# 9to1url/PairPhone

Hardware: AMD Instinct MI355X
Metric: MELPe-1200 channel-seconds encoded/sec (node) (higher is better)
Workload: dtype int16/int32 saturating fixed point; 1 GPU; config 4: 262144 channels per GPU, melpe_a per superframe (NPP x3 + MELPe-1200 analysis + 81-bit packing); channels_per_gpu=262144, channels_total=262144, parallelism=channel shards, 1 GPU(s), no collective

## Files before the change

### pairphone_amd/csrc/k_npp.hip

```cpp
#ifndef MELPE_NPP_WG_WAVES
#define MELPE_NPP_WG_WAVES 1
#endif
#ifndef MELPE_NPP_MATH_LDS
#define MELPE_NPP_MATH_LDS 1
#endif
#if MELPE_NPP_MATH_LDS
#define MELPE_MATH_LDS
#endif
#include "kern.h"
#include "npp_wave.h"
#include "dsp_eval.h"

MELPE_TU(npp)

#define NPP_WG (WAVE * MELPE_NPP_WG_WAVES)
#if MELPE_NPP_MATH_LDS
static_assert((160 * 1024 / (MELPE_NPP_WG_WAVES * sizeof(mlp::wv::NppWave) + MTAB_WORDS * sizeof(int16_t))) *
			      MELPE_NPP_WG_WAVES >= 16,
	      "16 NPP waves per CU (the register budget's four per SIMD)");
#define NPP_LDS_DYN (MTAB_WORDS * sizeof(int16_t))
#define NPP_TABLES_IN()                                                        \
	do {                                                                   \
		for (int i_ = threadIdx.x; i_ < MTAB_WORDS; i_ += blockDim.x) \
			s_mtab[i_] = g_tab[mtab_src(i_)];                     \
		__syncthreads();                                               \
	} while (0)
#else
#define NPP_LDS_DYN 0
#define NPP_TABLES_IN() (void) 0
#endif

#ifndef NPP_WAVES_PER_EU
#define NPP_WAVES_PER_EU 4
#endif
#define NPP_WPE __attribute__((amdgpu_waves_per_eu(NPP_WAVES_PER_EU)))

using namespace mlp::wv;

__global__ __launch_bounds__(NPP_WG) NPP_WPE void k_npp(EncState *enc, int16_t *sp, int frames, int stride,
					      const uint8_t *active, int n, int rate1200)
{
	__shared__ NppWave Ws[MELPE_NPP_WG_WAVES];
	NPP_TABLES_IN();
	const int w = __builtin_amdgcn_readfirstlane(threadIdx.x / WAVE), lane = threadIdx.x % WAVE;
	const int c = blockIdx.x * MELPE_NPP_WG_WAVES + w;
	if (c >= n || (active && !active[c]))
		return;
	NppWave &W = Ws[w];
	WvConst kc;
	wv_const_init(&kc, lane);
	wv_state_in(&W, &enc[c].npp, lane);
	int16_t *x = sp + (size_t) c * stride;
	for (int f = 0; f < frames; f++)
		wv_npp_frame(&W, &enc[c].npp, x + f * NPP_HOP, stride - f * NPP_HOP, rate1200 != 0, &kc, lane);
	wv_state_out(&enc[c].npp, &W, lane);
}

__global__ __launch_bounds__(NPP_WG) NPP_WPE void k_enc_npp(EncState *enc, int16_t *sp, const uint8_t *active,
						  int n)
{
	__shared__ NppWave Ws[MELPE_NPP_WG_WAVES];
	NPP_TABLES_IN();
	const int w = __builtin_amdgcn_readfirstlane(threadIdx.x / WAVE), lane = threadIdx.x % WAVE;
	const int c = blockIdx.x * MELPE_NPP_WG_WAVES + w;
	if (c >= n || (active && !active[c]))
		return;
	NppWave &W = Ws[w];
	WvConst kc;
	wv_const_init(&kc, lane);
	wv_state_in(&W, &enc[c].npp, lane);
	int16_t *x = sp + (size_t) c * BLOCK;
	for (int f = 0; f < NF; f++)
		wv_npp_frame(&W, &enc[c].npp, x + f * FRAME, BLOCK - f * FRAME, true, &kc, lane);
	wv_state_out(&enc[c].npp, &W, lane);
}

static unsigned npp_grid(int n)
{
	return (unsigned) ((n + MELPE_NPP_WG_WAVES - 1) / MELPE_NPP_WG_WAVES);
}

extern "C" int kl_npp(EncState *enc, int16_t *sp, int frames, int stride, const uint8_t *active,
		      int n, int rate1200, hipStream_t s)
{
	k_npp<<<npp_grid(n), NPP_WG, NPP_LDS_DYN, s>>>(enc, sp, frames, stride, active, n, rate1200);
	return (int) hipGetLastError();
}

static int launch_enc_npp(int waves, EncState *enc, int16_t *sp, const uint8_t *active, int n, hipStream_t s)
{
	k_enc_npp<<<npp_grid(waves), NPP_WG, NPP_LDS_DYN, s>>>(enc, sp, active, n);
	return (int) hipGetLastError();
}

extern "C" int kl_enc_npp(EncState *enc, int16_t *sp, const uint8_t *active, int n, hipStream_t s)
{
	return launch_enc_npp(n, enc, sp, active, n, s);
}

extern "C" size_t kl_npp_private(void)
{
	const size_t x = private_bytes((const void *) k_enc_npp), y = private_bytes((const void *) k_npp);
	return x > y ? x : y;
}

extern "C" int kl_npp_warm(int n, hipStream_t s)
{
	return launch_enc_npp(n, nullptr, nullptr, nullptr, 0, s);
}

__global__ __launch_bounds__(NPP_WG) void k_dsp_scalar_lds(int mode, const int32_t *args, int32_t *out, long n)
{
	NPP_TABLES_IN();
	long i = blockIdx.x * (long) blockDim.x + threadIdx.x;
	if (i >= n)
		return;
	const int32_t *a = args + 4 * i;
	out[i] = de_scalar(mode, a[0], a[1], a[2], a[3]);
}

__global__ __launch_bounds__(NPP_WG) void k_dsp_wave_fft(int mode, const int16_t *in, const int32_t *args,
							  int32_t *out, int n)
{
	__shared__ int16_t d[MELPE_NPP_WG_WAVES][DE_WV_IN];
	NPP_TABLES_IN();
	const int w = __builtin_amdgcn_readfirstlane(threadIdx.x / WAVE), lane = threadIdx.x % WAVE;
	const int c = blockIdx.x * MELPE_NPP_WG_WAVES + w;
	if (c >= n)
		return;
	WvConst kc;
	wv_const_init(&kc, lane);
	LANE_LOOP(k, DE_WV_IN)
		d[w][k] = in[(size_t) c * DE_WV_IN + k];
	wsync();
	const Word16 g = mode == 1 ? wv_fft_npp(d[w], (Word16) args[4 * (size_t) c], &kc, lane)
				   : wv_cfft256(d[w], &kc, lane);
	int32_t *o = out + (size_t) c * DE_WV_OUT;
	if (lane < DE_RET)
		o[lane] = lane == 0 ? g : 0;
	LANE_LOOP(k, DE_WV_IN)
		o[DE_RET + k] = d[w][k];
}

extern "C" int kl_dsp_scalar_lds(int mode, const int32_t *args, int32_t *out, long n, hipStream_t s)
{
	k_dsp_scalar_lds<<<(unsigned) ((n + NPP_WG - 1) / NPP_WG), NPP_WG, NPP_LDS_DYN, s>>>(mode, args, out, n);
	return (int) hipGetLastError();
}

extern "C" int kl_dsp_wave_fft(int mode, const int16_t *in, const int32_t *args, int32_t *out, int n,
			       hipStream_t s)
{
	k_dsp_wave_fft<<<npp_grid(n), NPP_WG, NPP_LDS_DYN, s>>>(mode, in, args, out, n);
	return (int) hipGetLastError();
}
```

### pairphone_amd/csrc/npp.h

```cpp
#ifndef MELPE_NPP_H
#define MELPE_NPP_H

#include <stddef.h>

#include "dsp.h"

namespace mlp {

#define NPP_WIN 256
#define NPP_HOP 180
#define NPP_OVL 76
#define NPP_NB 129
#define NPP_NMINWIN 8
#define NPP_LMINWIN 9
#define GM_MIN 3932
#define ENH_QK_MAX 32735
#define ENH_QK_MIN 33
#define NOISE_BIAS 23170

struct NppState {
	int16_t started;
	int16_t qk_started;
	int16_t pf_started;
	int16_t enh_i;
// ... 460 lines not shown
	}
	s1 = sub(norm_l(L), 1);
	Word16 t1 = extract_h(L_shl(L, s1));
	Word16 t = sub(sub(s4, s1), ns2_shift);
	w->var_rel[i] = divide_s(t1, ns2);
	if (cmp_shift(w->var_rel[i], t, 16384, 0) > 0)
		w->var_rel[i] = 16384;
	else
		w->var_rel[i] = shl(w->var_rel[i], t);
	if (w->var_rel[i] < 0)
		w->var_rel[i] = 0;
}

template <class SC>
MD Word16 npp_bias_scalars(NppState *s, const SC *w, Word32 vsum, Word16 *f1, Word16 *f2)
{
	vsum = L_shl(vsum, 1);
	vsum = L_sub(vsum, L_deposit_l(w->var_rel[0]));
	vsum = L_sub(vsum, L_deposit_l(w->var_rel[NPP_NB - 1]));
	s->var_rel_av = extract_l(L_shr(vsum, 8));
	if (s->var_rel_av < 0)
		s->var_rel_av = 0;
	Word16 vsq = mult(12288, sqrt_Q15(s->var_rel_av));
	vsq = add(8192, vsq);
	*f1 = extract_h(L_shl(L_mult(vsq, 16521), 1));
	*f2 = extract_h(L_shl(L_mult(vsq, 18643), 1));
	return vsq;
}

template <class SC>
MD void npp_bias2_bin(const NppState *s, const SC *w, int16_t &bsp, int16_t &bsh,
		      int16_t &bsub, int16_t &bsubsh, Word16 vsq, Word16 f1, Word16 f2, int i)
{
	Word32 L3 = L_mult(vsq, s->smoothedspect[i]);
	Word16 vr = w->var_rel[i];
	Word32 L4 = L_mult(vr, s->smoothedspect[i]);
	Word16 t = add(19543, shr(vr, 1));
	t = add(11656, shr(mult(vr, t), 1));
	Word32 L = L_mpy_ls(L_mpy_ls(L4, f1), t);
	L = L_add(L_shr(L3, 6), L_shr(L, 1));
	if (L < 1)
		L = 1;
	Word16 s1 = norm_l(L);
	bsp = extract_h(L_shl(L, s1));
	bsh = add(s->sm_shift[i], sub(8, s1));
	t = add(13968, shr(vr, 2));
	t = add(11909, shr(mult(vr, t), 1));
	L = L_mpy_ls(L_mpy_ls(L4, f2), t);
	L = L_add(L_shr(L3, 4), L_shr(L, 1));
	if (L < 1)
		L = 1;
	s1 = norm_l(L);
	bsub = extract_h(L_shl(L, s1));
	bsubsh = add(s->sm_shift[i], sub(6, s1));
}

MN void npp_bias_compensation(NppState *s, NppScratch *w, int16_t *bsp, int16_t *bsh,
			      int16_t *bsub, int16_t *bsubsh)
{
	Word32 vsum = 0;
	for (int i = 0; i < NPP_NB; i++) {
		npp_bias1_bin(s, w, i, w->alpha_var[i], w->noisespect2[i], w->noise2_shift[i]);
		vsum = L_add(vsum, L_deposit_l(w->var_rel[i]));
	}
	Word16 f1, f2;
	Word16 vsq = npp_bias_scalars(s, w, vsum, &f1, &f2);
	for (int i = 0; i < NPP_NB; i++)
		npp_bias2_bin(s, w, bsp[i], bsh[i], bsub[i], bsubsh[i], vsq, f1, f2, i);
}

MD Word16 npp_noise_slope(const NppState *s)
{
	if (s->var_rel_av > 5898)
		return 2703;
	if (s->var_rel_av < 983 || s->enh_i < 50)
		return 18022;
	if (s->var_rel_av < 1638)
		return 9011;
	if (s->var_rel_av < 1966)
		return 4506;
	return 2703;
}

MD void npp_min_search_bin(NppState *s, NppState *m, int16_t bsp, int16_t bsh, int16_t bsub,
			   int16_t bsubsh, Word16 slope, int i)
{
	if (s->minspec_counter == 0) {
		if (cmp_shift(bsp, bsh, s->act_min[i], s->act_min_shift[i]) < 0) {
			s->act_min[i] = bsp;
			s->act_min_shift[i] = bsh;
			m->act_min_sub[i] = bsub;
			m->act_min_sub_shift[i] = bsubsh;
			m->localflag[i] = 0;
		}
		m->circb[s->circb_index][i] = s->act_min[i];
		m->circb_shift[s->circb_index][i] = s->act_min_shift[i];
		Word16 t1 = m->circb[0][i], t2 = m->circb_shift[0][i];
		for (int k = 1; k < NPP_NMINWIN; k++)
			if (cmp_shift(m->circb[k][i], m->circb_shift[k][i], t1, t2) < 0) {
				t1 = m->circb[k][i];
				t2 = m->circb_shift[k][i];
			}
		m->circb_min[i] = t1;
		m->circb_min_shift[i] = t2;
		Word16 t = mult(slope, m->circb_min[i]);
		Word16 ts = add(m->circb_min_shift[i], 4);
		if (m->localflag[i] &&
		    cmp_shift(m->act_min_sub[i], m->act_min_sub_shift[i],
			      m->circb_min[i], m->circb_min_shift[i]) > 0 &&
		    cmp_shift(m->act_min_sub[i], m->act_min_sub_shift[i], t, ts) < 0) {
			m->circb_min[i] = m->act_min_sub[i];
			m->circb_min_shift[i] = m->act_min_sub_shift[i];
			for (int k = 0; k < NPP_NMINWIN; k++) {
				m->circb[k][i] = m->circb_min[i];
				m->circb_shift[k][i] = m->circb_min_shift[i];
			}
		}
		m->localflag[i] = 0;
	} else if (s->minspec_counter == 1) {
		s->act_min[i] = bsp;
		s->act_min_shift[i] = bsh;
		m->act_min_sub[i] = bsub;
		m->act_min_sub_shift[i] = bsubsh;
	} else {
		if (cmp_shift(bsp, bsh, s->act_min[i], s->act_min_shift[i]) < 0) {
			s->act_min[i] = bsp;
			s->act_min_shift[i] = bsh;
			m->act_min_sub[i] = bsub;
			m->act_min_sub_shift[i] = bsubsh;
			m->localflag[i] = 1;
		}
		if (cmp_shift(m->act_min_sub[i], m->act_min_sub_shift[i],
			      m->circb_min[i], m->circb_min_shift[i]) < 0) {
			m->circb_min[i] = m->act_min_sub[i];
			m->circb_min_shift[i] = m->act_min_sub_shift[i];
		}
		s->noisespect[i] = m->circb_min[i];
		s->noise_shift[i] = m->circb_min_shift[i];
		Word32 L = L_mult(NOISE_BIAS, s->noisespect[i]);
		if (L < 0x40000000L) {
			L = L_shl(L, 1);
			s->lambdaD_shift[i] = s->noise_shift[i];
		} else {
			s->lambdaD_shift[i] = add(s->noise_shift[i], 1);
		}
		s->lambdaD[i] = extract_h(L);
	}
}

MD void npp_min_search_post(NppState *s)
{
	if (s->minspec_counter == 0) {
		s->circb_index = add(s->circb_index, 1);
		if (s->circb_index == NPP_NMINWIN)
			s->circb_index = 0;
	}
	s->minspec_counter = add(s->minspec_counter, 1);
	if (s->minspec_counter == NPP_LMINWIN)
		s->minspec_counter = 0;
}

MN void npp_min_search(NppState *s, const int16_t *bsp, const int16_t *bsh,
		       const int16_t *bsub, const int16_t *bsubsh)
{
	Word16 slope = npp_noise_slope(s);
	for (int i = 0; i < NPP_NB; i++)
		npp_min_search_bin(s, s, bsp[i], bsh[i], bsub[i], bsubsh[i], slope, i);
	npp_min_search_post(s);
}

MN void npp_minstat_init(NppState *s)
{
	v_copy(s->smoothedspect, s->lambdaD, NPP_NB);
	v_scale(s->smoothedspect, NOISE_BIAS, NPP_NB);
	for (int k = 0; k < NPP_NMINWIN; k++) {
		v_copy(s->circb[k], s->smoothedspect, NPP_NB);
		v_copy(s->circb_shift[k], s->lambdaD_shift, NPP_NB);
	}
	v_copy(s->sm_shift, s->lambdaD_shift, NPP_NB);
	v_copy(s->act_min, s->smoothedspect, NPP_NB);
	v_copy(s->act_min_shift, s->lambdaD_shift, NPP_NB);
	v_copy(s->act_min_sub, s->smoothedspect, NPP_NB);
	v_copy(s->act_min_sub_shift, s->lambdaD_shift, NPP_NB);
	v_copy(s->noisespect, s->smoothedspect, NPP_NB);
	v_copy(s->noise_shift, s->lambdaD_shift, NPP_NB);
	for (int i = 0; i < NPP_NB; i++) {
		s->var_sp_av[i] = mult(s->smoothedspect[i], 20066);
		s->av_shift[i] = add(s->lambdaD_shift[i], 1);
		Word32 L = L_mult(s->smoothedspect[i], s->smoothedspect[i]);
		Word16 sh = norm_l(L);
		s->var_sp_2[i] = extract_h(L_shl(L, sh));
		s->av2_shift[i] = sub(shl(s->lambdaD_shift[i], 1), sub(sh, 1));
	}
	s->alphacorr = 29491;
}

MN void npp_enh_init(NppState *s, NppScratch *w, int16_t *noise)
{
	int16_t *yb = w->ybuf;
	int32_t ty[NPP_WIN + 2];
	window(noise, TB(sqrt_tukey_256_180), noise, NPP_WIN);
	Word16 mx = 1;
	for (int i = 0; i < NPP_WIN; i++) {
		Word16 t = abs_s(noise[i]);
		if (t > mx)
			mx = t;
	}
	Word16 sh = norm_s(mx);
	Word16 ash = sub(15, sh);
	v_zero(yb, 2 * NPP_WIN + 2);
	for (int i = 0; i < NPP_WIN; i++)
		yb[2 * i] = shl(noise[i], sh);
	Word16 g = fft_npp(yb, 1);
	ty[0] = L_shr(L_mult(yb[0], yb[0]), 1);
	ty[1] = 0;
	ty[NPP_WIN] = L_shr(L_mult(yb[NPP_WIN], yb[NPP_WIN]), 1);
	ty[NPP_WIN + 1] = 0;
	for (int i = 2; i < NPP_WIN - 1; i += 2) {
		ty[i + 1] = 0;
		ty[i] = L_shr(L_add(L_mult(yb[i], yb[i]), L_mult(yb[i + 1], yb[i + 1])), 1);
	}
	Word32 L = ty[0];
	for (int i = 1; i < NPP_WIN + 1; i++)
		if (L < ty[i])
			L = ty[i];
	sh = norm_l(L);
	for (int i = 0; i < NPP_WIN + 1; i++)
		yb[i] = extract_h(L_shl(ty[i], sh));
	sh = sub(shl(add(ash, g), 1), add(sh, 7));
	for (int i = 0; i < NPP_WIN / 2 - 1; i++) {
// ... 352 lines not shown
```

### pairphone_amd/csrc/npp_wave.h

```cpp
#ifndef MELPE_NPP_WAVE_H
#define MELPE_NPP_WAVE_H

#include "npp.h"

namespace mlp {
namespace wv {

#define WV 64
#define LANE_LOOP(i, n) for (int i = lane; i < (n); i += WV)
#define BIN_LOOP(t, i) \
	_Pragma("unroll") for (int t = 0, i = lane; t < 3; t++, i += WV) if (i < NPP_NB)

#define BIN_PASSES(t, i, ...) \
	_Pragma("unroll") for (int t = 0, i = lane; t < 3; t++, i += WV) if (i < NPP_NB) { \
		__VA_ARGS__ \
	}
__device__ __forceinline__ void wsync()
{
#if defined(MELPE_NPP_WG_WAVES) && MELPE_NPP_WG_WAVES > 1
	__builtin_amdgcn_fence(__ATOMIC_RELEASE, "wavefront");
	__builtin_amdgcn_wave_barrier();
	__builtin_amdgcn_fence(__ATOMIC_ACQUIRE, "wavefront");
#else
	__syncthreads();
// ... 171 lines not shown
		o[6] = sub(v[2], v[7]);
		o[3] = sub(v[3], v[6]);
		o[7] = add(v[3], v[6]);
		m = 0;
		for (int k = 0; k < 8; k++) {
			d0[i + k] = o[k];
			m = max(m, (int) abs_s(o[k]));
		}
	}
	int16_t *d = d0 - 1;
	int st = 0;
#pragma unroll
	for (int mmax = 8; mmax < 512; mmax *= 2, st++) {
		Word16 mx = (Word16) wmax(m);
		sc = 0;
		if (mx > 16383) {
			g += 2;
			sc = 2;
		} else if (mx > 8191) {
			g += 1;
			sc = 1;
		}
		wsync();
		int istep = 2 * mmax;
		int half = mmax / 2;
		m = 0;
		for (int t = 0; t < 2; t++) {
			int b = lane + WV * t;
			int k = b % half, blk = b / half;
			int i = 1 + 2 * k + blk * istep;
			int jj = i + mmax;
			Word16 wr = (Word16) (kc->tw[st][t] & 0xffff);
			Word16 wi = (Word16) (kc->tw[st][t] >> 16);
			Word16 pr = shr(d[i], sc), qr = shr(d[jj], sc);
			Word16 pi = shr(d[i + 1], sc), qi = shr(d[jj + 1], sc);
			Word32 tr = L_add(L_mult(wr, qr), L_mult(wi, qi));
			tr = L_add(tr, L_shl(0x80, 8));
			tr = L_shl(L_shr(tr, 16), 16);
			Word32 ti = L_sub(L_mult(wi, qr), L_mult(wr, qi));
			ti = L_add(ti, L_shl(0x80, 8));
			ti = L_shl(L_shr(ti, 16), 16);
			Word16 o0 = extract_h(L_add(L_deposit_h(pr), tr));
			Word16 o1 = extract_h(L_sub(L_deposit_h(pr), tr));
			Word16 o2 = extract_h(L_sub(L_deposit_h(pi), ti));
			Word16 o3 = extract_h(L_add(L_deposit_h(pi), ti));
			d[i] = o0;
			d[jj] = o1;
			d[i + 1] = o2;
			d[jj + 1] = o3;
			m = max(m, max(max((int) abs_s(o0), (int) abs_s(o1)),
				       max((int) abs_s(o2), (int) abs_s(o3))));
		}
	}
	wsync();
	return g;
}

MD Word16 wv_fft_npp(int16_t *d, Word16 dir, const WvConst *kc, int lane)
{
	Word16 g = wv_cfft256(d, kc, lane);
	if (dir < 0) {
		for (int n = 1 + lane; n < 128; n += WV) {
			int16_t t = d[2 * n];
			d[2 * n] = d[2 * (256 - n)];
			d[2 * (256 - n)] = t;
			t = d[2 * n + 1];
			d[2 * n + 1] = d[2 * (256 - n) + 1];
			d[2 * (256 - n) + 1] = t;
		}
		wsync();
	}
	return g;
}

MD void wv_mirror(int16_t *yb, int lane)
{
	LANE_LOOP(i, NPP_WIN / 2 - 1) {
		yb[NPP_WIN + 2 * i + 2] = yb[NPP_WIN - 2 * i - 2];
		yb[NPP_WIN + 2 * i + 3] = negate(yb[NPP_WIN - 2 * i - 1]);
	}
	wsync();
}

MD void wv_minstat_init(NppState *s, NppState *m, int lane)
{
	LANE_LOOP(i, NPP_NB) {
		Word16 sp = mult(s->lambdaD[i], NOISE_BIAS);
		Word16 ls = s->lambdaD_shift[i];
		s->smoothedspect[i] = sp;
		for (int k = 0; k < NPP_NMINWIN; k++) {
			m->circb[k][i] = sp;
			m->circb_shift[k][i] = ls;
		}
		s->sm_shift[i] = ls;
		s->act_min[i] = sp;
		s->act_min_shift[i] = ls;
		m->act_min_sub[i] = sp;
		m->act_min_sub_shift[i] = ls;
		s->noisespect[i] = sp;
		s->noise_shift[i] = ls;
		s->var_sp_av[i] = mult(sp, 20066);
		s->av_shift[i] = add(ls, 1);
		Word32 L = L_mult(sp, sp);
		Word16 sh = norm_l(L);
		s->var_sp_2[i] = extract_h(L_shl(L, sh));
		s->av2_shift[i] = sub(shl(ls, 1), sub(sh, 1));
	}
	s->alphacorr = 29491;
}

MD void wv_enh_init(NppWave *W, int16_t *noise, const WvConst *kc, int lane, NppState *m)
{
	NppState *s = wv_S(W);
	int16_t *yb = W->w.ybuf;
	u32_alias *ty = W->ty_init;
	int mx = 0;
#pragma unroll
	LANE_LOOP(i, NPP_WIN) {
		noise[i] = mult(kc->win[i >> 6], noise[i]);
		mx = max(mx, (int) abs_s(noise[i]));
	}
	mx = max(1, wmax(mx));
	Word16 sh = norm_s((Word16) mx);
	Word16 ash = sub(15, sh);
	LANE_LOOP(i, NPP_WIN + 1) {
		yb[2 * i] = (i < NPP_WIN) ? shl(noise[i], sh) : (int16_t) 0;
		yb[2 * i + 1] = 0;
	}
	wsync();
	Word16 g = wv_fft_npp(yb, 1, kc, lane);
	int Lm = INT32_MIN;
	LANE_LOOP(p, NPP_NB) {
		int i = 2 * p;
		Word32 v;
		if (p == 0 || p == NPP_NB - 1)
			v = L_shr(L_mult(yb[i], yb[i]), 1);
		else
			v = L_shr(L_add(L_mult(yb[i], yb[i]), L_mult(yb[i + 1], yb[i + 1])), 1);
		ty[i] = (uint32_t) v;
		ty[i + 1] = 0;
		Lm = max(Lm, (int) v);
		if (p != NPP_NB - 1)
			Lm = max(Lm, 0);
	}
	Word32 L = wmax(Lm);
	wsync();
	sh = norm_l(L);
	LANE_LOOP(i, NPP_WIN + 1)
		yb[i] = extract_h(L_shl((Word32) ty[i], sh));
	sh = sub(shl(add(ash, g), 1), add(sh, 7));
	wsync();
	wv_mirror(yb, lane);
	g = wv_fft_npp(yb, -1, kc, lane);
	sh = add(sh, g);
	sh = sub(sh, 8);
	mx = 0;
	LANE_LOOP(i, NPP_WIN) {
		noise[i] = yb[2 * i];
		mx = max(mx, (int) abs_s(noise[i]));
	}
	mx = wmax(mx);
	Word16 t = norm_s((Word16) mx);
	sh = sub(sh, t);
	const int16_t *wf = TB(wtr_front);
	LANE_LOOP(i, NPP_WIN) {
		Word16 v = shl(noise[i], t);
		if (i >= 1 && i < 32)
			v = mult(v, wf[i]);
		else if (i >= NPP_WIN - 32 + 1)
			v = mult(v, wf[NPP_WIN - i]);
		else if (i >= 32)
			v = 0;
		noise[i] = v;
	}
	wsync();
	LANE_LOOP(i, NPP_WIN + 1) {
		yb[2 * i] = (i < NPP_WIN) ? noise[i] : (int16_t) 0;
		yb[2 * i + 1] = 0;
	}
	wsync();
	g = wv_fft_npp(yb, 1, kc, lane);
	Word16 nsh = add(sh, g);
	int part = 0;
	LANE_LOOP(p, NPP_NB) {
		Word16 y = yb[2 * p];
		if (y < 0)
			y = 0;
		Word32 Ld = L_add(L_shl(L_mult(181, y), 7), 2);
		Word16 ns = norm_l(Ld);
		s->lambdaD[p] = extract_h(L_shl(Ld, ns));
		s->lambdaD_shift[p] = add(nsh, sub(1, ns));
		part += (p == 0 || p == NPP_NB - 1) ? L_shr(Ld, 8) : L_shr(Ld, 7);
	}
	L = wsum(part);
	sh = norm_l(L);
	s->n_pwr = extract_h(L_shl(L, sh));
	s->n_pwr_shift = sub(add(nsh, 1), sh);
	s->SN_LT = divide_s(14648, s->n_pwr);
	s->SN_LT_shift = sub(22, s->n_pwr_shift);
	wv_minstat_init(s, m, lane);
	wsync();
}

MD void wv_gain_scan_serial(const int16_t *gk, const int16_t *gks, int lane, int *acc_out, int *sh_out,
			    int *mn_out, int *ms_out, bool sum)
{
	int gk0 = gk[lane], gk1 = gk[lane + 64], gk2 = gk[NPP_NB - 1];
	int gs0 = gks[lane], gs1 = gks[lane + 64], gs2 = gks[NPP_NB - 1];
	int acc, sh2;
	int mn, ms;
	{
		int g = __builtin_amdgcn_readlane(gk0, 0), e = __builtin_amdgcn_readlane(gs0, 0);
		acc = g << 7;
		sh2 = e - 1;
		mn = g;
		ms = e;
	}
	auto shc = [](int k) { return k < 0 ? 0 : (k > 31 ? 31 : k); };
	auto step = [&](int g, int e, int ee) {
		int d = ms - e;
		int a1 = d > 0 ? mn : mn >> shc(-d);
		int b1 = d > 0 ? g >> shc(d) : g;
		bool take = a1 < b1;
		mn = take ? g : mn;
		ms = take ? e : ms;
		if (sum) {
			int t = sh2 - ee;
			int n = t - 7;
			int term = n >= 0 ? g >> shc(n) : g << shc(-n);
			int accb = (acc >> shc(-t)) + (g << 7);
			acc = t > 0 ? acc + term : accb;
			sh2 = t > 0 ? sh2 : ee;
		}
	};
	#pragma unroll 2
	for (int i = 1; i < 64; i++) {
		int e = __builtin_amdgcn_readlane(gs0, i);
		step(__builtin_amdgcn_readlane(gk0, i), e, e);
	}
	#pragma unroll 2
	for (int i = 0; i < 64; i++) {
		int e = __builtin_amdgcn_readlane(gs1, i);
		step(__builtin_amdgcn_readlane(gk1, i), e, e);
	}
	step(gk2, gs2, gs2 - 1);
	*acc_out = acc;
	*sh_out = sh2;
	*mn_out = mn;
	*ms_out = ms;
}

MD void wv_gain_scan(const int16_t *gk, const int16_t *gks, int lane, Word16 *gav, Word16 *gavs,
		     Word16 *gmax, Word16 *gmaxs)
{
	const int g0 = gk[lane], g1 = gk[lane + 64], g2 = gk[NPP_NB - 1];
	const int e0 = gks[lane], e1 = gks[lane + 64], e2 = gks[NPP_NB - 1];
	const int a0 = lane == 0 ? e0 - 1 : e0, a2 = e2 - 1;
	const int M0 = wscan_max(a0);
	const int M1 = max(__builtin_amdgcn_readlane(M0, 63), wscan_max(e1));
	const int M2 = max(__builtin_amdgcn_readlane(M1, 63), a2);
	const int dmax = M2 - __builtin_amdgcn_readlane(a0, 0);
	int acc, sh2, mn, ms;
	bool serial_sum = dmax > 32;
	if (!serial_sum) {
		auto term = [](int g, int t) { return t >= 7 ? g >> (t - 7 > 31 ? 31 : t - 7) : g << (7 - t); };
		const int t0 = term(g0, M0 - a0), t1 = term(g1, M1 - e1), t2 = term(g2, M2 - a2);
		const int d0 = M2 - M0, d1 = M2 - M1;
		auto ip = [](int t, int d) { return d >= 32 ? 0 : t >> d; };
		auto fp = [](int t, int d) {
			return d == 0 ? 0u : (uint32_t) ((uint64_t) (uint32_t) t << (32 - d));
		};
		const uint32_t f0 = fp(t0, d0), f1 = fp(t1, d1);
		const int si = wsum(ip(t0, d0) + ip(t1, d1)) + t2;
		const int slo = wsum((int) ((f0 & 0xffffu) + (f1 & 0xffffu)));
		const int shi = wsum((int) ((f0 >> 16) + (f1 >> 16)));
		acc = si + ((shi + (slo >> 16)) >> 16);
		sh2 = M2;
	}
	const int emx = max(wmax(max(e0, e1)), e2), emn = min(-wmax(-min(e0, e1)), e2);
	if (serial_sum || emx > 100 || emn < -100) {
		int a, s2;
		wv_gain_scan_serial(gk, gks, lane, &a, &s2, &mn, &ms, serial_sum);
		if (serial_sum) {
			acc = a;
			sh2 = s2;
		}
	} else {
		const float v0 = ldexpf((float) g0, e0), v1 = ldexpf((float) g1, e1), v2 = ldexpf((float) g2, e2);
		const int E0 = wscan_max(e0);
		const int E1 = max(__builtin_amdgcn_readlane(E0, 63), wscan_max(e1));
		const int E2 = max(__builtin_amdgcn_readlane(E1, 63), e2);
		const float I0 = wscan_maxf(v0);
		const float I1 = fmaxf(__int_as_float(__builtin_amdgcn_readlane(__float_as_int(I0), 63)), wscan_maxf(v1));
		const float I2 = fmaxf(__int_as_float(__builtin_amdgcn_readlane(__float_as_int(I1), 63)), v2);
		const bool c0 = v0 > I0 - ldexpf(1.0f, E0 + 1) && lane != 0;
		const bool c1 = v1 > I1 - ldexpf(1.0f, E1 + 1);
		const bool c2 = v2 > I2 - ldexpf(1.0f, E2 + 1);
		uint64_t m0 = __ballot(c0), m1 = __ballot(c1);
		mn = __builtin_amdgcn_readlane(g0, 0);
		ms = __builtin_amdgcn_readlane(e0, 0);
		auto shc = [](int k) { return k < 0 ? 0 : (k > 31 ? 31 : k); };
		auto step = [&](int g, int e) {
			int d = ms - e;
			int x = d > 0 ? mn : mn >> shc(-d);
			int y = d > 0 ? g >> shc(d) : g;
			bool take = x < y;
			mn = take ? g : mn;
			ms = take ? e : ms;
		};
		while (m0) {
			const int k = __builtin_ctzll(m0);
			m0 &= m0 - 1;
			step(__builtin_amdgcn_readlane(g0, k), __builtin_amdgcn_readlane(e0, k));
		}
		while (m1) {
			const int k = __builtin_ctzll(m1);
			m1 &= m1 - 1;
			step(__builtin_amdgcn_readlane(g1, k), __builtin_amdgcn_readlane(e1, k));
		}
		if (c2)
			step(g2, e2);
	}
	Word32 L = acc;
	if (L == 0)
		L = 1;
	Word16 t1 = norm_l(L);
	*gav = extract_h(L_shl(L, t1));
	*gavs = add(sub((Word16) sh2, t1), 2);
	*gmax = (Word16) mn;
	*gmaxs = (Word16) ms;
}

MD void wv_process_frame(NppWave *W, NppState *m, const int16_t *in, int16_t *out, const WvConst *kc,
			 int lane)
{
	PROF_SCOPE(34);
	NppState *s = wv_S(W);
	NppScratchW *w = &W->w;
	int16_t *yb = w->ybuf;
	int16_t *GainD = W->GainD, *gk = W->gk, *gks = W->gks;
	Word16 sh, t, t1, t2, t3, t4;
	Word32 L;

	if (!s->pf_started) {
		LANE_LOOP(i, NPP_NB) {
			s->agal[i] = 0;
			s->agal_shift[i] = 0;
			s->ksi[i] = GM_MIN;
			s->ksi_shift[i] = 0;
			s->qk[i] = ENH_QK_MAX;
			s->Gain[i] = GM_MIN;
		}
		s->YY_LT = 0;
		s->YY_LT_shift = 0;
		s->SN_LT0 = s->SN_LT;
		s->SN_LT0_shift = s->SN_LT_shift;
		s->pf_started = 1;
	}
	LANE_LOOP(i, NPP_NB)
		GainD[i] = GM_MIN;
	if (s->enh_i < 50)
		s->enh_i = (int16_t) (s->enh_i + 1);

	int16_t *analy = W->buf;
	Word16 g, Ysh, YYavs;
	{
	PROF_SCOPE(60);
	int mx = 0;
#pragma unroll
	LANE_LOOP(i, NPP_WIN) {
		analy[i] = mult(kc->win[i >> 6], in[i]);
		mx = max(mx, (int) abs_s(analy[i]));
	}
	mx = max(1, wmax(mx));
	sh = norm_s((Word16) mx);
	Word16 ash = sub(15, sh);
	LANE_LOOP(i, NPP_WIN + 1) {
		yb[2 * i] = (i < NPP_WIN) ? shl(analy[i], sh) : (int16_t) 0;
		yb[2 * i + 1] = 0;
	}
	wsync();
	g = wv_fft_npp(yb, 1, kc, lane);
	Ysh = add(ash, g);
	YYavs = shl(Ysh, 1);
	}
	int maxs = SW_MIN_;
	int part = 0;
	int16_t ymag[3] = {0, 0, 0}, ymag_sh[3] = {0, 0, 0};
	{
	PROF_SCOPE(53);
	BIN_PASSES(t, i, {
		Word32 v;
		if (i == 0)
			v = L_mult(yb[0], yb[0]);
		else if (i == NPP_NB - 1)
			v = L_mult(yb[NPP_WIN], yb[NPP_WIN]);
		else
			v = L_add(L_mult(yb[2 * i], yb[2 * i]), L_mult(yb[2 * i + 1], yb[2 * i + 1]));
		if (v < 1)
			v = 1;
		Word16 n = norm_l(v);
		w->YY[i] = extract_h(L_shl(v, n));
		w->YY_shift[i] = sub(YYavs, n);
		maxs = max(maxs, (int) w->YY_shift[i]);
	})
	maxs = wmax(maxs);
	BIN_PASSES(t, i, {
		Word16 y = w->YY[i], ys = w->YY_shift[i];
		if (ys & 1) {
			y = shr(y, 1);
			ys = add(ys, 1);
		}
		ymag[t] = sqrt_Q15(y);
		ymag_sh[t] = shr(ys, 1);
		w->YY_shift[i] = sub(w->YY_shift[i], 8);
		Word32 st = npp_spec_term(w->YY, w->YY_shift, (Word16) maxs, i);
		part += st;
	})
	L = wsum(part);
	}
	if (L == 0)
		L = 1;
	t1 = norm_l(L);
	Word16 YY_av = extract_h(L_shl(L, t1));
	Word16 YY_av_shift = sub(add((Word16) maxs, 1), t1);

	{
	PROF_SCOPE(36);
	maxs = SW_MIN_;
	BIN_PASSES(t, i, { maxs = max(maxs, (int) s->sm_shift[i]); })
	maxs = wmax(maxs);
	part = 0;
	BIN_PASSES(t, i, {
		Word32 st = npp_spec_term(s->smoothedspect, s->sm_shift, (Word16) maxs, i);
		part += st;
	})
	L = wsum(part);
	Word16 amin;
	Word16 anum = npp_sm_period_scalars(s, (Word16) maxs, L, YY_av, YY_av_shift, &amin);
	part = 0;
	{
	PROF_SCOPE(54);
	BIN_PASSES(t, i, {
		int16_t ns2, ns2sh, av;
		npp_sm_period_bin(s, w, anum, amin, i, ns2, ns2sh, av);
		npp_bias1_bin(s, w, i, av, ns2, ns2sh);
		part += w->var_rel[i];
	})
	}
	Word32 vsum = wsum(part);
	wsync();
	Word16 f1, f2;
	Word16 vsq = npp_bias_scalars(s, w, vsum, &f1, &f2);
	Word16 slope = npp_noise_slope(s);
	{
	PROF_SCOPE(55);
	BIN_PASSES(t, i, {
		int16_t bsp, bsh, bsub, bsubsh;
		npp_bias2_bin(s, w, bsp, bsh, bsub, bsubsh, vsq, f1, f2, i);
		npp_min_search_bin(s, m, bsp, bsh, bsub, bsubsh, slope, i);
		gk[i] = divide_s(shr(w->YY[i], 1), s->lambdaD[i]);
		gks[i] = sub(add(w->YY_shift[i], 1), s->lambdaD_shift[i]);
	})
	}
	wsync();
	npp_min_search_post(s);
	}

	Word16 gav, gavs, gmax, gmaxs;
	{
	PROF_SCOPE(37);
	wv_gain_scan(gk, gks, lane, &gav, &gavs, &gmax, &gmaxs);
	}
	bool nflag = false;
	if (cmp_shift(gmax, gmaxs, 18102, 6) < 0 && cmp_shift(gav, gavs, 23170, 1) < 0) {
		nflag = true;
		t1 = mult(s->n_pwr, 23170);
		t2 = add(s->n_pwr_shift, 2);
		if (cmp_shift(YY_av, YY_av_shift, t1, t2) > 0)
			nflag = false;
	}

	{
	PROF_SCOPE(38);
	if (s->enh_i == 1) {
		BIN_LOOP(t, i) {
			Word32 v = L_mult(ymag[t], GM_MIN);
			Word16 n = norm_l(v);
			s->agal[i] = extract_h(L_shl(v, n));
			s->agal_shift[i] = sub(ymag_sh[t], n);
		}
	} else {
		{
		PROF_SCOPE(56);
		BIN_PASSES(t, i, { npp_ksi_bin(s, gk, gks, i); })
		}
		t1 = mult(29491, s->Ksi_min_var);
		t2 = mult(3277, npp_ksi_min_adapt(nflag, GM_MIN, s->SN_LT, s->SN_LT_shift));
		Word16 kmv = add(t1, t2);
		s->Ksi_min_var = kmv;
		sh = norm_s(kmv);
		t1 = shl(kmv, sh);
		Word16 nsh = negate(sh);
		BIN_PASSES(t, i, {
			if (cmp_shift(s->ksi[i], s->ksi_shift[i], t1, nsh) < 0) {
				s->ksi[i] = t1;
				s->ksi_shift[i] = nsh;
			}
			s->qk[i] = ENH_QK_MAX;
		})
		if (!nflag) {
			if (cmp_shift(gav, gavs, 23170, 1) > 0) {
				L = L_mult(s->YY_LT, 32023);
				sh = norm_l(L);
				t1 = extract_h(L_shl(L, sh));
				t2 = sub(s->YY_LT_shift, sh);
				L = L_mult(YY_av, 745);
				sh = norm_l(L);
				t3 = extract_h(L_shl(L, sh));
				t4 = sub(YY_av_shift, sh);
				t1 = shr(t1, 1);
				t3 = shr(t3, 1);
				sh = sub(t2, t4);
				Word16 yl, yls;
				if (sh > 0) {
					yl = add(t1, shr(t3, sh));
					yls = t2;
				} else {
					yl = add(shl(t1, sh), t3);
					yls = t4;
				}
				yls = add(yls, 1);
				if (sub(yl, s->n_pwr) > 0) {
					yl = shr(yl, 1);
					yls = add(yls, 1);
				}
				s->YY_LT = yl;
				s->YY_LT_shift = yls;
				Word16 sn = divide_s(yl, s->n_pwr);
				Word16 sns = sub(yls, s->n_pwr_shift);
				if (cmp_shift(sn, sns, SW_MAX_, 0) < 0) {
					sn = s->SN_LT0;
					sns = s->SN_LT0_shift;
// ... 3 lines not shown
					sn = extract_h(L_shl(L, sh));
					sns = sub(sns, sh);
				}
				s->SN_LT = sn;
				s->SN_LT_shift = sns;
				s->SN_LT0 = sn;
				s->SN_LT0_shift = sns;
			}
			bool first = !s->qk_started;
			PROF_SCOPE(57);
			BIN_PASSES(t, i, {
				npp_compute_qk_bin(s, s->qk, gk, gks, 19273, first, i);
				if (s->qk[i] > ENH_QK_MAX)
					s->qk[i] = ENH_QK_MAX;
				else if (s->qk[i] < ENH_QK_MIN)
					s->qk[i] = ENH_QK_MIN;
			})
			s->qk_started = 1;
		}
		PROF_SCOPE(58);
		BIN_PASSES(t, i, {
			int16_t vk, vksh;
			npp_gain_log_mmse_bin(s, vk, vksh, s->qk, s->Gain, gk, gks, i);
			GainD[i] = s->Gain[i];
			npp_gain_mod_bin(s, vk, vksh, s->qk, GainD, i);
			Word32 v = L_mult(GainD[i], ymag[t]);
			Word16 n = norm_l(v);
			s->agal[i] = extract_h(L_shl(v, n));
			s->agal_shift[i] = sub(ymag_sh[t], n);
		})
	}
	}
	wsync();
	{
	PROF_SCOPE(59);
	int lm = 0;
	Word32 tyr[5];
#pragma unroll
	for (int t = 0; t < 5; t++) {
		int i = lane + WV * t;
		tyr[t] = 0;
		if (i < NPP_WIN + 2) {
			Word32 v = L_mult(yb[i], GainD[i / 2]);
			tyr[t] = v;
			lm = max(lm, (int) L_abs(v));
		}
	}
	Word32 Lmax = wmax(lm);
	sh = norm_l(Lmax);
#pragma unroll
	for (int t = 0; t < 5; t++) {
		int i = lane + WV * t;
		if (i < NPP_WIN + 2)
			yb[i] = extract_h(L_shl(tyr[t], sh));
	}
	sh = sub(Ysh, sh);
	wsync();
	wv_mirror(yb, lane);
	g = wv_fft_npp(yb, -1, kc, lane);
	sh = add(sh, g);
	sh = sub(sh, 8);
	Word16 osh = sub(sh, 15);
#pragma unroll
	LANE_LOOP(i, NPP_WIN)
		out[i] = mult(shl(yb[2 * i], osh), kc->win[i >> 6]);
	}
	maxs = SW_MIN_;
	BIN_PASSES(t, i, { maxs = max(maxs, (int) s->lambdaD_shift[i]); })
	maxs = wmax(maxs);
	part = 0;
	BIN_PASSES(t, i, {
		Word32 st = npp_spec_term(s->lambdaD, s->lambdaD_shift, (Word16) maxs, i);
		part += st;
	})
	L = wsum(part);
	if (L == 0)
		L = 1;
	sh = norm_l(L);
	s->n_pwr = extract_h(L_shl(L, sh));
	s->n_pwr_shift = add(sub((Word16) maxs, sh), 1);
	wsync();
}

MD void wv_npp_frame(NppWave *W, NppState *m, int16_t *x, int avail, bool rate1200, const WvConst *kc,
		     int lane)
{
	PROF_SCOPE(0);
	NppState *s = wv_S(W);
	if (!s->started) {
		int16_t *noise = W->buf;
		LANE_LOOP(i, NPP_WIN) {
			int16_t v = 0;
			if (rate1200)
				v = i < avail ? x[i] : (int16_t) 0;
			else if (i >= NPP_OVL)
				v = x[i - NPP_OVL];
			noise[i] = v;
		}
		wsync();
		wv_enh_init(W, noise, kc, lane, m);
		LANE_LOOP(i, NPP_WIN)
			s->speech_in[i] = 0;
		s->started = 1;
		wsync();
	}
	LANE_LOOP(i, NPP_OVL)
		s->speech_in[i] = s->speech_in[NPP_HOP + i];
	wsync();
	LANE_LOOP(i, NPP_HOP)
		s->speech_in[NPP_OVL + i] = x[i];
	wsync();
	wv_process_frame(W, m, s->speech_in, W->buf, kc, lane);
	LANE_LOOP(i, NPP_OVL) {
		Word16 o = add(W->buf[i], s->overlap[i]);
		s->overlap[i] = W->buf[NPP_HOP + i];
		W->buf[i] = o;
	}
	wsync();
	LANE_LOOP(i, NPP_HOP)
		x[i] = W->buf[i];
	wsync();
}

MD void wv_state_in(NppWave *W, const NppState *g, int lane)
{
	PROF_SCOPE(35);
	const u32_alias *src = (const u32_alias *) g;
	u32_alias *dst = W->s_hot;
	LANE_LOOP(i, (int) (NPP_HOT_BYTES / 4))
		dst[i] = src[i];
	wsync();
}

MD void wv_state_out(NppState *g, const NppWave *W, int lane)
{
	PROF_SCOPE(35);
	wsync();
	const u32_alias *src = W->s_hot;
	u32_alias *dst = (u32_alias *) g;
	LANE_LOOP(i, (int) (NPP_HOT_BYTES / 4))
		dst[i] = src[i];
}

}
}

#endif
```

Measured before the change: 544,100 channel-s/s.

## Keep NPP minimum-statistics per-bin state in registers and use buffer loads for ring

Moves the per-bin minimum-search fields (act_min_sub, circb_min, localflag) out of global memory into packed per-lane registers for the whole multi-frame kernel, loading them once at kernel start and storing once at the end. The circular buffer is read only on ring-update frames via raw buffer loads/stores with a wave-uniform ring offset, writing a single slot instead of rewriting it. The hot-state copy into LDS is also widened to 16-byte vector loads and stores. The aim is to cut repeated global-memory traffic per frame, at the cost of extra VGPR pressure that may lower occupancy under the four-waves-per-SIMD budget.

```diff
diff --git a/pairphone_amd/csrc/k_npp.hip b/pairphone_amd/csrc/k_npp.hip
--- a/pairphone_amd/csrc/k_npp.hip
+++ b/pairphone_amd/csrc/k_npp.hip
@@ -37,6 +37,7 @@
 
 using namespace mlp::wv;
 
+
 __global__ __launch_bounds__(NPP_WG) NPP_WPE void k_npp(EncState *enc, int16_t *sp, int frames, int stride,
 					      const uint8_t *active, int n, int rate1200)
 {
@@ -49,11 +50,14 @@
 	NppWave &W = Ws[w];
 	WvConst kc;
 	wv_const_init(&kc, lane);
+	NppMinRegs R;
+	wv_min_in(R, &enc[c].npp, lane);
 	wv_state_in(&W, &enc[c].npp, lane);
 	int16_t *x = sp + (size_t) c * stride;
 	for (int f = 0; f < frames; f++)
-		wv_npp_frame(&W, &enc[c].npp, x + f * NPP_HOP, stride - f * NPP_HOP, rate1200 != 0, &kc, lane);
+		wv_npp_frame(&W, &enc[c].npp, R, x + f * NPP_HOP, stride - f * NPP_HOP, rate1200 != 0, &kc, lane);
 	wv_state_out(&enc[c].npp, &W, lane);
+	wv_min_out(&enc[c].npp, R, lane);
 }
 
 __global__ __launch_bounds__(NPP_WG) NPP_WPE void k_enc_npp(EncState *enc, int16_t *sp, const uint8_t *active,
@@ -68,11 +72,14 @@
 	NppWave &W = Ws[w];
 	WvConst kc;
 	wv_const_init(&kc, lane);
+	NppMinRegs R;
+	wv_min_in(R, &enc[c].npp, lane);
 	wv_state_in(&W, &enc[c].npp, lane);
 	int16_t *x = sp + (size_t) c * BLOCK;
 	for (int f = 0; f < NF; f++)
-		wv_npp_frame(&W, &enc[c].npp, x + f * FRAME, BLOCK - f * FRAME, true, &kc, lane);
+		wv_npp_frame(&W, &enc[c].npp, R, x + f * FRAME, BLOCK - f * FRAME, true, &kc, lane);
 	wv_state_out(&enc[c].npp, &W, lane);
+	wv_min_out(&enc[c].npp, R, lane);
 }
 
 static unsigned npp_grid(int n)
diff --git a/pairphone_amd/csrc/npp.h b/pairphone_amd/csrc/npp.h
--- a/pairphone_amd/csrc/npp.h
+++ b/pairphone_amd/csrc/npp.h
@@ -566,61 +566,66 @@
 	return 2703;
 }
 
-MD void npp_min_search_bin(NppState *s, NppState *m, int16_t bsp, int16_t bsh, int16_t bsub,
-			   int16_t bsubsh, Word16 slope, int i)
-{
+struct NppMinBin {
+	int16_t act_min_sub, act_min_sub_shift;
+	int16_t localflag;
+	int16_t circb_min, circb_min_shift;
+};
+
+MD bool npp_min_search_val(NppState *s, NppMinBin &b, const int16_t *ring, const int16_t *ring_sh,
+			   int16_t bsp, int16_t bsh, int16_t bsub, int16_t bsubsh, Word16 slope, int i)
+{
+	bool fill = false;
 	if (s->minspec_counter == 0) {
 		if (cmp_shift(bsp, bsh, s->act_min[i], s->act_min_shift[i]) < 0) {
 			s->act_min[i] = bsp;
 			s->act_min_shift[i] = bsh;
-			m->act_min_sub[i] = bsub;
-			m->act_min_sub_shift[i] = bsubsh;
-			m->localflag[i] = 0;
-		}
-		m->circb[s->circb_index][i] = s->act_min[i];
-		m->circb_shift[s->circb_index][i] = s->act_min_shift[i];
-		Word16 t1 = m->circb[0][i], t2 = m->circb_shift[0][i];
-		for (int k = 1; k < NPP_NMINWIN; k++)
-			if (cmp_shift(m->circb[k][i], m->circb_shift[k][i], t1, t2) < 0) {
-				t1 = m->circb[k][i];
-				t2 = m->circb_shift[k][i];
+			b.act_min_sub = bsub;
+			b.act_min_sub_shift = bsubsh;
+			b.localflag = 0;
+		}
+		const int ci = s->circb_index;
+		Word16 t1 = ci == 0 ? s->act_min[i] : ring[0];
+		Word16 t2 = ci == 0 ? s->act_min_shift[i] : ring_sh[0];
+		for (int k = 1; k < NPP_NMINWIN; k++) {
+			Word16 r1 = ci == k ? s->act_min[i] : ring[k];
+			Word16 r2 = ci == k ? s->act_min_shift[i] : ring_sh[k];
+			if (cmp_shift(r1, r2, t1, t2) < 0) {
+				t1 = r1;
+				t2 = r2;
 			}
-		m->circb_min[i] = t1;
-		m->circb_min_shift[i] = t2;
-		Word16 t = mult(slope, m->circb_min[i]);
-		Word16 ts = add(m->circb_min_shift[i], 4);
-		if (m->localflag[i] &&
-		    cmp_shift(m->act_min_sub[i], m->act_min_sub_shift[i],
-			      m->circb_min[i], m->circb_min_shift[i]) > 0 &&
-		    cmp_shift(m->act_min_sub[i], m->act_min_sub_shift[i], t, ts) < 0) {
-			m->circb_min[i] = m->act_min_sub[i];
-			m->circb_min_shift[i] = m->act_min_sub_shift[i];
-			for (int k = 0; k < NPP_NMINWIN; k++) {
-				m->circb[k][i] = m->circb_min[i];
-				m->circb_shift[k][i] = m->circb_min_shift[i];
-			}
-		}
-		m->localflag[i] = 0;
+		}
+		b.circb_min = t1;
+		b.circb_min_shift = t2;
+		Word16 t = mult(slope, b.circb_min);
+		Word16 ts = add(b.circb_min_shift, 4);
+		if (b.localflag &&
+		    cmp_shift(b.act_min_sub, b.act_min_sub_shift, b.circb_min, b.circb_min_shift) > 0 &&
+		    cmp_shift(b.act_min_sub, b.act_min_sub_shift, t, ts) < 0) {
+			b.circb_min = b.act_min_sub;
+			b.circb_min_shift = b.act_min_sub_shift;
+			fill = true;
+		}
+		b.localflag = 0;
 	} else if (s->minspec_counter == 1) {
 		s->act_min[i] = bsp;
 		s->act_min_shift[i] = bsh;
-		m->act_min_sub[i] = bsub;
-		m->act_min_sub_shift[i] = bsubsh;
+		b.act_min_sub = bsub;
+		b.act_min_sub_shift = bsubsh;
 	} else {
 		if (cmp_shift(bsp, bsh, s->act_min[i], s->act_min_shift[i]) < 0) {
 			s->act_min[i] = bsp;
 			s->act_min_shift[i] = bsh;
-			m->act_min_sub[i] = bsub;
-			m->act_min_sub_shift[i] = bsubsh;
-			m->localflag[i] = 1;
-		}
-		if (cmp_shift(m->act_min_sub[i], m->act_min_sub_shift[i],
-			      m->circb_min[i], m->circb_min_shift[i]) < 0) {
-			m->circb_min[i] = m->act_min_sub[i];
-			m->circb_min_shift[i] = m->act_min_sub_shift[i];
-		}
-		s->noisespect[i] = m->circb_min[i];
-		s->noise_shift[i] = m->circb_min_shift[i];
+			b.act_min_sub = bsub;
+			b.act_min_sub_shift = bsubsh;
+			b.localflag = 1;
+		}
+		if (cmp_shift(b.act_min_sub, b.act_min_sub_shift, b.circb_min, b.circb_min_shift) < 0) {
+			b.circb_min = b.act_min_sub;
+			b.circb_min_shift = b.act_min_sub_shift;
+		}
+		s->noisespect[i] = b.circb_min;
+		s->noise_shift[i] = b.circb_min_shift;
 		Word32 L = L_mult(NOISE_BIAS, s->noisespect[i]);
 		if (L < 0x40000000L) {
 			L = L_shl(L, 1);
@@ -630,6 +635,40 @@
 		}
 		s->lambdaD[i] = extract_h(L);
 	}
+	return fill;
+}
+
+MD void npp_min_ring_store(const NppState *s, NppState *m, const NppMinBin &b, bool fill, int i)
+{
+	if (fill) {
+		for (int k = 0; k < NPP_NMINWIN; k++) {
+			m->circb[k][i] = b.circb_min;
+			m->circb_shift[k][i] = b.circb_min_shift;
+		}
+	} else if (s->minspec_counter == 0) {
+		m->circb[s->circb_index][i] = s->act_min[i];
+		m->circb_shift[s->circb_index][i] = s->act_min_shift[i];
+	}
+}
+
+MD void npp_min_search_bin(NppState *s, NppState *m, int16_t bsp, int16_t bsh, int16_t bsub,
+			   int16_t bsubsh, Word16 slope, int i)
+{
+	NppMinBin b = {m->act_min_sub[i], m->act_min_sub_shift[i], m->localflag[i], m->circb_min[i],
+		       m->circb_min_shift[i]};
+	int16_t ring[NPP_NMINWIN] = {0}, ring_sh[NPP_NMINWIN] = {0};
+	if (s->minspec_counter == 0)
+		for (int k = 0; k < NPP_NMINWIN; k++) {
+			ring[k] = m->circb[k][i];
+			ring_sh[k] = m->circb_shift[k][i];
+		}
+	bool fill = npp_min_search_val(s, b, ring, ring_sh, bsp, bsh, bsub, bsubsh, slope, i);
+	npp_min_ring_store(s, m, b, fill, i);
+	m->act_min_sub[i] = b.act_min_sub;
+	m->act_min_sub_shift[i] = b.act_min_sub_shift;
+	m->localflag[i] = b.localflag;
+	m->circb_min[i] = b.circb_min;
+	m->circb_min_shift[i] = b.circb_min_shift;
 }
 
 MD void npp_min_search_post(NppState *s)
diff --git a/pairphone_amd/csrc/npp_wave.h b/pairphone_amd/csrc/npp_wave.h
--- a/pairphone_amd/csrc/npp_wave.h
+++ b/pairphone_amd/csrc/npp_wave.h
@@ -277,21 +277,74 @@
 	wsync();
 }
 
-MD void wv_minstat_init(NppState *s, NppState *m, int lane)
-{
-	LANE_LOOP(i, NPP_NB) {
+struct NppMinRegs {
+	unsigned sub[3];
+	unsigned cmin[3];
+	unsigned flag;
+};
+
+typedef __amdgpu_buffer_rsrc_t MinRec;
+MD MinRec wv_min_rec(const NppState *m)
+{
+	return __builtin_amdgcn_make_buffer_rsrc((char *) const_cast<NppState *>(m) + NPP_HOT_BYTES, 0,
+						 (int) (sizeof(NppState) - NPP_HOT_BYTES), 0x00020000);
+}
+#define MOFF(lane, t, field) (2 * (lane) + (int) (offsetof(NppState, field) - NPP_HOT_BYTES + 2 * WV * (t)))
+#define MRING_OFF(lane, t, field, k) (MOFF(lane, t, field) + (int) ((k) * NPP_NB * sizeof(int16_t)))
+__device__ __forceinline__ int16_t mld(MinRec r, int off, int soff = 0)
+{
+	return (int16_t) __builtin_amdgcn_raw_buffer_load_b16(r, off, soff, 0);
+}
+__device__ __forceinline__ void mst(MinRec r, int off, int16_t v, int soff = 0)
+{
+	__builtin_amdgcn_raw_buffer_store_b16(v, r, off, soff, 0);
+}
+
+__device__ __forceinline__ unsigned pack16(int16_t lo, int16_t hi)
+{
+	return (unsigned) (uint16_t) lo | (unsigned) (uint16_t) hi << 16;
+}
+
+MD void wv_min_in(NppMinRegs &R, const NppState *m, int lane)
+{
+	const MinRec r = wv_min_rec(m);
+	R.flag = 0;
+	_Pragma("unroll") for (int t = 0; t < 3; t++)
+		R.sub[t] = R.cmin[t] = 0;
+	BIN_PASSES(t, i, {
+		R.sub[t] = pack16(mld(r, MOFF(lane, t, act_min_sub)), mld(r, MOFF(lane, t, act_min_sub_shift)));
+		R.cmin[t] = pack16(mld(r, MOFF(lane, t, circb_min)), mld(r, MOFF(lane, t, circb_min_shift)));
+		R.flag |= (unsigned) (mld(r, MOFF(lane, t, localflag)) != 0) << t;
+	})
+}
+
+MD void wv_min_out(NppState *m, const NppMinRegs &R, int lane)
+{
+	const MinRec r = wv_min_rec(m);
+	BIN_PASSES(t, i, {
+		mst(r, MOFF(lane, t, act_min_sub), (int16_t) R.sub[t]);
+		mst(r, MOFF(lane, t, act_min_sub_shift), (int16_t) (R.sub[t] >> 16));
+		mst(r, MOFF(lane, t, circb_min), (int16_t) R.cmin[t]);
+		mst(r, MOFF(lane, t, circb_min_shift), (int16_t) (R.cmin[t] >> 16));
+		mst(r, MOFF(lane, t, localflag), (int16_t) (R.flag >> t & 1));
+	})
+}
+
+MD void wv_minstat_init(NppState *s, NppState *m, NppMinRegs &R, int lane)
+{
+	const MinRec r = wv_min_rec(m);
+	BIN_PASSES(t, i, {
 		Word16 sp = mult(s->lambdaD[i], NOISE_BIAS);
 		Word16 ls = s->lambdaD_shift[i];
 		s->smoothedspect[i] = sp;
 		for (int k = 0; k < NPP_NMINWIN; k++) {
-			m->circb[k][i] = sp;
-			m->circb_shift[k][i] = ls;
+			mst(r, MRING_OFF(lane, t, circb, k), sp);
+			mst(r, MRING_OFF(lane, t, circb_shift, k), ls);
 		}
 		s->sm_shift[i] = ls;
 		s->act_min[i] = sp;
 		s->act_min_shift[i] = ls;
-		m->act_min_sub[i] = sp;
-		m->act_min_sub_shift[i] = ls;
+		R.sub[t] = pack16(sp, ls);
 		s->noisespect[i] = sp;
 		s->noise_shift[i] = ls;
 		s->var_sp_av[i] = mult(sp, 20066);
@@ -300,11 +353,11 @@
 		Word16 sh = norm_l(L);
 		s->var_sp_2[i] = extract_h(L_shl(L, sh));
 		s->av2_shift[i] = sub(shl(ls, 1), sub(sh, 1));
-	}
+	})
 	s->alphacorr = 29491;
 }
 
-MD void wv_enh_init(NppWave *W, int16_t *noise, const WvConst *kc, int lane, NppState *m)
+MD void wv_enh_init(NppWave *W, int16_t *noise, const WvConst *kc, int lane, NppState *m, NppMinRegs &R)
 {
 	NppState *s = wv_S(W);
 	int16_t *yb = W->w.ybuf;
@@ -393,7 +446,7 @@
 	s->n_pwr_shift = sub(add(nsh, 1), sh);
 	s->SN_LT = divide_s(14648, s->n_pwr);
 	s->SN_LT_shift = sub(22, s->n_pwr_shift);
-	wv_minstat_init(s, m, lane);
+	wv_minstat_init(s, m, R, lane);
 	wsync();
 }
 
@@ -526,8 +579,8 @@
 	*gmaxs = (Word16) ms;
 }
 
-MD void wv_process_frame(NppWave *W, NppState *m, const int16_t *in, int16_t *out, const WvConst *kc,
-			 int lane)
+MD void wv_process_frame(NppWave *W, NppState *m, NppMinRegs &R, const int16_t *in, int16_t *out,
+			 const WvConst *kc, int lane)
 {
 	PROF_SCOPE(34);
 	NppState *s = wv_S(W);
@@ -648,12 +701,36 @@
 	Word16 f1, f2;
 	Word16 vsq = npp_bias_scalars(s, w, vsum, &f1, &f2);
 	Word16 slope = npp_noise_slope(s);
+	const bool ring_frame = __builtin_amdgcn_readfirstlane((int) s->minspec_counter) == 0;
+	const int ring_at = __builtin_amdgcn_readfirstlane((int) s->circb_index) * (int) (NPP_NB * sizeof(int16_t));
+	const MinRec r = wv_min_rec(m);
 	{
 	PROF_SCOPE(55);
 	BIN_PASSES(t, i, {
 		int16_t bsp, bsh, bsub, bsubsh;
+		int16_t ring[NPP_NMINWIN] = {0}, ring_sh[NPP_NMINWIN] = {0};
+		if (ring_frame) {
+			_Pragma("unroll") for (int k = 0; k < NPP_NMINWIN; k++) {
+				ring[k] = mld(r, MRING_OFF(lane, t, circb, k));
+				ring_sh[k] = mld(r, MRING_OFF(lane, t, circb_shift, k));
+			}
+		}
 		npp_bias2_bin(s, w, bsp, bsh, bsub, bsubsh, vsq, f1, f2, i);
-		npp_min_search_bin(s, m, bsp, bsh, bsub, bsubsh, slope, i);
+		NppMinBin b = {(int16_t) R.sub[t], (int16_t) (R.sub[t] >> 16), (int16_t) (R.flag >> t & 1),
+			       (int16_t) R.cmin[t], (int16_t) (R.cmin[t] >> 16)};
+		bool fill = npp_min_search_val(s, b, ring, ring_sh, bsp, bsh, bsub, bsubsh, slope, i);
+		if (fill) {
+			_Pragma("unroll") for (int k = 0; k < NPP_NMINWIN; k++) {
+				mst(r, MRING_OFF(lane, t, circb, k), b.circb_min);
+				mst(r, MRING_OFF(lane, t, circb_shift, k), b.circb_min_shift);
+			}
+		} else if (ring_frame) {
+			mst(r, MRING_OFF(lane, t, circb, 0), s->act_min[i], ring_at);
+			mst(r, MRING_OFF(lane, t, circb_shift, 0), s->act_min_shift[i], ring_at);
+		}
+		R.sub[t] = pack16(b.act_min_sub, b.act_min_sub_shift);
+		R.cmin[t] = pack16(b.circb_min, b.circb_min_shift);
+		R.flag = (R.flag & ~(1u << t)) | (unsigned) (b.localflag != 0) << t;
 		gk[i] = divide_s(shr(w->YY[i], 1), s->lambdaD[i]);
 		gks[i] = sub(add(w->YY_shift[i], 1), s->lambdaD_shift[i]);
 	})
@@ -823,8 +900,8 @@
 	wsync();
 }
 
-MD void wv_npp_frame(NppWave *W, NppState *m, int16_t *x, int avail, bool rate1200, const WvConst *kc,
-		     int lane)
+MD void wv_npp_frame(NppWave *W, NppState *m, NppMinRegs &R, int16_t *x, int avail, bool rate1200,
+		     const WvConst *kc, int lane)
 {
 	PROF_SCOPE(0);
 	NppState *s = wv_S(W);
@@ -839,7 +916,7 @@
 			noise[i] = v;
 		}
 		wsync();
-		wv_enh_init(W, noise, kc, lane, m);
+		wv_enh_init(W, noise, kc, lane, m, R);
 		LANE_LOOP(i, NPP_WIN)
 			s->speech_in[i] = 0;
 		s->started = 1;
@@ -851,7 +928,7 @@
 	LANE_LOOP(i, NPP_HOP)
 		s->speech_in[NPP_OVL + i] = x[i];
 	wsync();
-	wv_process_frame(W, m, s->speech_in, W->buf, kc, lane);
+	wv_process_frame(W, m, R, s->speech_in, W->buf, kc, lane);
 	LANE_LOOP(i, NPP_OVL) {
 		Word16 o = add(W->buf[i], s->overlap[i]);
 		s->overlap[i] = W->buf[NPP_HOP + i];
@@ -863,13 +940,21 @@
 	wsync();
 }
 
+typedef uint32_t u32x4_alias __attribute__((ext_vector_type(4), may_alias, aligned(16)));
+static_assert(NPP_HOT_BYTES % 16 == 0 && sizeof(EncState) % 16 == 0 && offsetof(EncState, npp) % 16 == 0,
+	      "NppState hot part copied in 16-byte pieces");
 MD void wv_state_in(NppWave *W, const NppState *g, int lane)
 {
 	PROF_SCOPE(35);
-	const u32_alias *src = (const u32_alias *) g;
+	const u32x4_alias *src = (const u32x4_alias *) g;
 	u32_alias *dst = W->s_hot;
-	LANE_LOOP(i, (int) (NPP_HOT_BYTES / 4))
-		dst[i] = src[i];
+	LANE_LOOP(i, (int) (NPP_HOT_BYTES / 16)) {
+		u32x4_alias v = src[i];
+		dst[4 * i] = v.x;
+		dst[4 * i + 1] = v.y;
+		dst[4 * i + 2] = v.z;
+		dst[4 * i + 3] = v.w;
+	}
 	wsync();
 }
 
@@ -878,9 +963,15 @@
 	PROF_SCOPE(35);
 	wsync();
 	const u32_alias *src = W->s_hot;
-	u32_alias *dst = (u32_alias *) g;
-	LANE_LOOP(i, (int) (NPP_HOT_BYTES / 4))
-		dst[i] = src[i];
+	u32x4_alias *dst = (u32x4_alias *) g;
+	LANE_LOOP(i, (int) (NPP_HOT_BYTES / 16)) {
+		u32x4_alias v;
+		v.x = src[4 * i];
+		v.y = src[4 * i + 1];
+		v.z = src[4 * i + 2];
+		v.w = src[4 * i + 3];
+		dst[i] = v;
+	}
 }
 
 }
```

Result: faster. 558,500 channel-s/s, median of 6 (+2.6%).
